# nihaomiao/WACV23_TSNet

Measured on AMD Instinct MI355X. Metric: retargeted frames/sec at bs=4, 256x256, n_source=3; max-abs delta vs ref, higher is better.
Workload: dtype f32 (convolutions: fp16 x 2 split of the scaled fp32 operands, 3 exact MFMA products, two-level fp32 accumulate; fp32-class accuracy); 1 GPU; TSNet(label_nc=2,n_blocks=0,n_downsampling=3,n_source=3) forward, fp32, B=4 per GPU, 256x256 (BASELINE.json configs[1]); global_batch=4, parallelism=replicas x1 (batch-sharded, weights broadcast once)

## Files before the change

include/tsnet_abi.h:

```cpp
#ifndef TSNET_ABI_H
#define TSNET_ABI_H

#include <stddef.h>
#include <stdint.h>

#ifdef __cplusplus
extern "C" {
#endif

#define TSNET_ABI_VERSION 5
#define TSNET_MAX_SOURCES 8

enum {
    TSNET_OK = 0,
    TSNET_ERR_ARG = -1,
    TSNET_ERR_WEIGHT = -2,
    TSNET_ERR_HIP = -3,
    TSNET_ERR_NOMEM = -4
};

typedef struct tsnet_engine* tsnet_handle;

typedef struct tsnet_cfg {
    int label_nc;
// ... 122 lines not shown
                       float* y, float* alpha, float* beta, void* stream);
int tsnet_op_finalize_stats(const double* part, int N, int S, int C, int HW, float* alpha, float* beta, void* stream);
int tsnet_op_fuse_tail(const float* src_fea, const float* tar_fea, const float* y2, const float* alpha, const float* beta,
                       int B, int K, int SB, int P, int C1, float* zbar, void* stream);
int tsnet_op_flow_k_slots(const float* tar_fea, const float* src_fea, const float* tar_bbox, const float* src_bbox,
                          int B, int K, int h, int w, int C, int H, int W, float* flow, int variant, int repeat, float* ms_out,
                          const int* slots, int n_src, void* stream);
int tsnet_op_warp_k_slots(const float* src_fea, const float* flow, int B, int K, int h, int w, int C, float* out,
                          const int* slots, int n_src, void* stream);
int tsnet_op_add_stats_slots(const float* x, const float* add, int add_nmod, int N, int HW, int C,
                             float* y, float* alpha, float* beta, const int* slots, int n_src, void* stream);
int tsnet_op_fuse_tail_slots(const float* src_fea, const float* tar_fea, const float* y2, const float* alpha, const float* beta,
                             int B, int K, int P, int C1, float* zbar, const int* slots, int n_src, void* stream);
int tsnet_op_pack_input(const float* const* img, const float* const* lbl, int S, int B, int H, int W, int L, int nimg, int Cp, int coords,
                        const float* img_div, float* out, unsigned int* amax, void* stream);
int tsnet_op_pack_input_u8(const uint8_t* const* img, const uint8_t* const* lbl, const uint8_t* const* bbox, int S, int B, int H, int W, int L,
                           int nimg, int Cp, int coords, const float* img_div, const float* mean_bgr, float* out, float* bbox_out,
                           unsigned int* amax, void* stream);
int tsnet_op_upsample2x_st(const float* x, const float* alpha, const float* beta, int relu,
                           int N, int H, int W, int C, int x_bf16, int y_bf16, float* y, void* stream);
int tsnet_op_patch_warp(const float* const* src_img, const float* div, const float* flow, int K, int B, int H, int W, int h, int w, float* out,
                        void* stream);
int tsnet_op_train_tail(float* x, const float* tar_img, const float* pg, const float* sg, int K, int B, int H, int W, int P, int C,
                        int fore_x0, int fore_x1, const float* bg, float* gen_mean, float* gen_std, float* ref_mean, float* ref_std,
                        float* losses, void* stream);
const char* tsnet_op_last_error(void);

int tsnet_frame_stats(const float* x, int B, int C, int HW, float div, float* mean, float* std_unbiased, void* stream);
int tsnet_demo_postprocess(const float* rec, int B, int H, int W, const float* gen_mean, const float* gen_std,
                           const float* ref_mean, const float* ref_std, const float* img_mean_over_255,
                           unsigned char* out_rgb, void* stream);

int tsnet_fit_face_curves(const double* keypoints, int F, double* curves);
int tsnet_raster_face(const double* keypoints, const double* curves, int F, int h, int w, int bw, unsigned char* edges, unsigned char* bbox, void* stream);
int tsnet_vl2ch(const float* labels, int B, int HW, int num_classes, float* out, void* stream);

int tsnet_face_adapt_stats(const double* kp, int F, double* stats);
int tsnet_face_adapt_apply(const double* stats, double* kp, int F);
int tsnet_smooth_keypoints(const double* in, int F, int P, double* out);

int tsnet_resize_label(const unsigned char* in, int F, int h, int w, int OH, int OW, const double* wts_rows, int lw_rows,
                       const double* wts_cols, int lw_cols, float* out, void* stream);
int tsnet_fit_pose_curves(const double* pts, int F, int flags, double* curves);
int tsnet_raster_pose(const double* pts, const double* curves, int F, int h, int w, int win_x0, int win_y0, int win_x1, int win_y1, int flags,
                      unsigned char* labels, void* stream);
int tsnet_label_bbox(const unsigned char* labels, int F, int h, int w, unsigned char* bbox, void* stream);
int tsnet_resize_pad(const unsigned char* in, int F, int h, int w, const int* ytab, const int* xtab, int oh, int ow,
                     int pad_top, int pad_left, int OH, int OW, int binarise, float* out, void* stream);

int tsnet_bench_conv(int N, int H, int W, int Cin, int Cout, int ksize, int stride, int pad, int pad_mode, int norm,
                     int variant, int iters, float* ms_out, void* stream);

void tsnet_debug_counters(int64_t out[4], int reset);

void tsnet_linspace(int n, float* out);
void tsnet_coord_table(int H, int W, float* out);

int tsnet_bicubic_taps(int n_in, int n_out);
int tsnet_bicubic_table(int n_in, int n_out, int* first, int* count, int* coef);
int tsnet_prepare_frames(const unsigned char* frames, int F, int h, int w, int x0, int y0, int x1, int y1,
                         const int* xfirst, const int* xcount, const int* xcoef, int xtaps,
                         const int* yfirst, const int* ycount, const int* ycoef, int ytaps,
                         int oh, int ow, int pad_top, int pad_left, int OH, int OW, const float* mean_bgr, float* out, void* stream);
int tsnet_prepare_frames_u8(const unsigned char* frames, int F, int h, int w, int x0, int y0, int x1, int y1,
                            const int* xfirst, const int* xcount, const int* xcoef, int xtaps,
                            const int* yfirst, const int* ycount, const int* ycoef, int ytaps,
                            int oh, int ow, int pad_top, int pad_left, int OH, int OW, unsigned char* out, void* stream);

int tsnet_paste_frames(const unsigned char* gen, const unsigned char* mask, int F, int GH, int GW, int sx0, int sy0, int sx1, int sy1,
                       const int* xfirst, const int* xcount, const int* xcoef, int xtaps,
                       const int* yfirst, const int* ycount, const int* ycoef, int ytaps,
                       unsigned char* frames, int h, int w, int x0, int y0, int x1, int y1, void* stream);

int tsnet_prepare_frames_boxes(const unsigned char* frames, int F, int h, int w, const int* boxes_host, const int* boxes_dev,
                               const int* pool, int pool_len, int oh, int ow, int pad_top, int pad_left, int OH, int OW,
                               const float* mean_bgr, float* out, void* stream);
int tsnet_prepare_frames_boxes_u8(const unsigned char* frames, int F, int h, int w, const int* boxes_host, const int* boxes_dev,
                                  const int* pool, int pool_len, int oh, int ow, int pad_top, int pad_left, int OH, int OW,
                                  unsigned char* out, void* stream);
int tsnet_paste_frames_boxes(const unsigned char* gen, const unsigned char* mask, int F, int GH, int GW, int sx0, int sy0, int sx1, int sy1,
                             const int* boxes_host, const int* boxes_dev, const int* pool, int pool_len,
                             unsigned char* frames, int h, int w, void* stream);

int tsnet_face_labels_boxes(const double* keypoints, const double* curves, int F, const int* desc_host, const int* desc_dev,
                            const double* pool, int pool_len, int bw, void* workspace, long long workspace_len, int OH, int OW,
                            float* labels, float* masks, void* stream);
int tsnet_face_labels_boxes_u8(const double* keypoints, const double* curves, int F, const int* desc_host, const int* desc_dev,
                               const double* pool, int pool_len, int bw, void* workspace, long long workspace_len, int OH, int OW,
                               unsigned char* labels, unsigned char* masks, void* stream);

int tsnet_gaussian_box_params(float radius, int passes, int* box_radius, unsigned* ww, unsigned* fw);
int tsnet_blur_mask(const unsigned char* in, int F, int H, int W, const int* rect, float radius_x, float radius_y, int flags,
                    unsigned char* out, unsigned char* tmp, void* stream);

#ifdef __cplusplus
}
#endif
#endif
```

wacv23_tsnet_amd/_lib.py:

```python
from __future__ import annotations

import ctypes as C
import os

import torch

_HERE = os.path.dirname(os.path.abspath(__file__))
LIB_PATH = os.path.join(_HERE, "lib", "libtsnet_hip.so")
MAX_SOURCES = 8
TIMING_CLASSES = 9
TIMING_NAMES = ("conv", "stats", "elementwise", "flow", "warp", "pack", "upsample", "other", "conv_res")

ABI_SYMBOLS = (
    "tsnet_abi_version", "tsnet_create", "tsnet_load_weights", "tsnet_finalize", "tsnet_destroy",
    "tsnet_last_error", "tsnet_num_params", "tsnet_param_info", "tsnet_packed_weights",
    "tsnet_forward", "tsnet_set_source_divisors", "tsnet_set_sources", "tsnet_set_sources_shared", "tsnet_forward_target", "tsnet_train_extras", "tsnet_stage_ptr",
    "tsnet_forward_macs", "tsnet_timing_enable", "tsnet_timing_read",
    "tsnet_op_conv2d", "tsnet_op_conv2d_cat", "tsnet_op_head", "tsnet_op_instnorm_stats", "tsnet_op_norm_act", "tsnet_op_upsample2x",
    "tsnet_op_flow", "tsnet_op_flow_k", "tsnet_flow_plan", "tsnet_op_warp", "tsnet_op_warp_k", "tsnet_op_warp_k_shared", "tsnet_op_add_stats", "tsnet_op_finalize_stats", "tsnet_op_fuse_tail", "tsnet_op_pack_input", "tsnet_op_upsample2x_st", "tsnet_op_last_error", "tsnet_frame_stats", "tsnet_demo_postprocess", "tsnet_fit_face_curves", "tsnet_raster_face", "tsnet_vl2ch", "tsnet_fit_pose_curves", "tsnet_raster_pose", "tsnet_label_bbox", "tsnet_resize_pad", "tsnet_resize_label", "tsnet_bench_conv", "tsnet_debug_counters", "tsnet_linspace", "tsnet_coord_table",
    "tsnet_bicubic_taps", "tsnet_bicubic_table", "tsnet_prepare_frames",
    "tsnet_face_adapt_stats", "tsnet_face_adapt_apply", "tsnet_smooth_keypoints",
    "tsnet_bank_capacity", "tsnet_bank_put", "tsnet_forward_bank",
    "tsnet_op_flow_k_slots", "tsnet_op_warp_k_slots", "tsnet_op_add_stats_slots", "tsnet_op_fuse_tail_slots",
    "tsnet_forward_u8", "tsnet_set_sources_u8", "tsnet_forward_target_u8", "tsnet_bank_put_u8", "tsnet_forward_bank_u8",
    "tsnet_op_pack_input_u8", "tsnet_prepare_frames_u8",
    "tsnet_paste_frames",
    "tsnet_prepare_frames_boxes", "tsnet_prepare_frames_boxes_u8", "tsnet_paste_frames_boxes",
    "tsnet_face_labels_boxes", "tsnet_face_labels_boxes_u8",
    "tsnet_op_upconv2d", "tsnet_op_conv2d_epi",
    "tsnet_op_patch_warp", "tsnet_op_train_tail",
    "tsnet_gaussian_box_params", "tsnet_blur_mask",
)


class TsnetCfg(C.Structure):
    _fields_ = [
        ("label_nc", C.c_int), ("n_blocks", C.c_int), ("n_downsampling", C.c_int), ("n_source", C.c_int),
        ("ngf", C.c_int), ("enc_blocks", C.c_int), ("addcoords", C.c_int), ("pose_composite", C.c_int),
        ("pose_mean", C.c_float * 3), ("height", C.c_int), ("width", C.c_int), ("max_batch", C.c_int), ("operand_mode", C.c_int),
    ]


_fp = C.POINTER(C.c_float)
_vp = C.c_void_p
CONV_EPI_INFO = 8


class TsnetConvEpi(C.Structure):
    _fields_ = [
        ("stats", C.c_int), ("repeat", C.c_int), ("part", _vp), ("part_capacity", C.c_longlong), ("alpha", _vp), ("beta", _vp),
        ("counters", _vp), ("counters_nonzero_out", C.POINTER(C.c_int)), ("addend", _vp), ("add_nmod", C.c_int), ("amax_out", _vp),
        ("in_amax", _vp), ("bound_add", C.c_float), ("x_bf16", C.c_int), ("y_bf16", C.c_int), ("info_out", C.POINTER(C.c_int)),
    ]


def bind(lib: C.CDLL) -> C.CDLL:
    lib.tsnet_abi_version.restype = C.c_int
    lib.tsnet_create.argtypes = [C.POINTER(TsnetCfg), C.POINTER(_vp)]
    lib.tsnet_load_weights.argtypes = [_vp, C.c_char_p, _vp, C.POINTER(C.c_int64), C.c_int]
    lib.tsnet_finalize.argtypes = [_vp, _vp]
    lib.tsnet_destroy.argtypes = [_vp]
    lib.tsnet_destroy.restype = None
    lib.tsnet_last_error.argtypes = [_vp]
    lib.tsnet_last_error.restype = C.c_char_p
    lib.tsnet_num_params.argtypes = [_vp]
    lib.tsnet_param_info.argtypes = [_vp, C.c_int, C.POINTER(C.c_char_p), C.POINTER(C.c_int64), C.POINTER(C.c_int)]
    lib.tsnet_packed_weights.argtypes = [_vp, C.POINTER(_vp), C.POINTER(C.c_size_t)]
    pp = C.POINTER(_vp)
    lib.tsnet_forward.argtypes = [_vp, pp, pp, pp, _vp, _vp, _vp, _vp, C.c_int, _vp]
    lib.tsnet_set_source_divisors.argtypes = [_vp, _fp, C.c_int]
    lib.tsnet_set_sources.argtypes = [_vp, pp, pp, pp, C.c_int, _vp]
    if hasattr(lib, "tsnet_set_sources_shared"):
        lib.tsnet_set_sources_shared.argtypes = [_vp, pp, pp, pp, _vp]
    lib.tsnet_forward_target.argtypes = [_vp, _vp, _vp, _vp, _vp, C.c_int, _vp]
    lib.tsnet_train_extras.argtypes = [_vp, pp, _vp, C.c_int, _vp, _vp, _vp]
    lib.tsnet_stage_ptr.argtypes = [_vp, C.c_char_p, C.POINTER(_vp), C.POINTER(C.c_size_t)]
    lib.tsnet_forward_macs.argtypes = [_vp, C.c_int]
    lib.tsnet_forward_macs.restype = C.c_double
    lib.tsnet_timing_enable.argtypes = [_vp, C.c_int]
    lib.tsnet_timing_read.argtypes = [_vp, C.POINTER(C.c_double), C.POINTER(C.c_int64), C.c_int]
    lib.tsnet_op_conv2d.argtypes = [_vp, C.c_int, C.c_int, C.c_int, C.c_int, _vp, _vp, C.c_int, C.c_int, C.c_int,
                                    C.c_int, C.c_int, _vp, _vp, C.c_int, C.c_float, C.c_int, C.c_int, C.c_int, _vp, _vp]
    lib.tsnet_op_conv2d_cat.argtypes = [_vp, _vp] + [C.c_int] * 6 + [_vp, _vp] + [C.c_int] * 5 + [C.c_float, C.c_int, _vp, _vp]
    lib.tsnet_op_head.argtypes = [_vp, C.c_int, C.c_int, C.c_int, C.c_int, _vp, _vp, _vp, _vp, C.c_int, _fp, _vp, _vp]
    lib.tsnet_op_instnorm_stats.argtypes = [_vp, C.c_int, C.c_int, C.c_int, _vp, _vp, _vp]
    lib.tsnet_op_norm_act.argtypes = [_vp, _vp, _vp, C.c_int, _vp, C.c_int, C.c_int, C.c_int, _vp, _vp]
    lib.tsnet_op_upsample2x.argtypes = [_vp, _vp, _vp, C.c_int, C.c_int, C.c_int, C.c_int, C.c_int, _vp, _vp]
    lib.tsnet_resize_label.argtypes = [_vp, C.c_int, C.c_int, C.c_int, C.c_int, C.c_int, _vp, C.c_int, _vp, C.c_int, _vp, _vp]
    lib.tsnet_op_flow.argtypes = [_vp, _vp, _vp, _vp, C.c_int, C.c_int, C.c_int, C.c_int, C.c_int, C.c_int, _vp, _vp]
    lib.tsnet_op_flow_k.argtypes = [_vp, _vp, _vp, _vp] + [C.c_int] * 7 + [_vp, C.c_int, C.c_int, _fp, _vp]
    lib.tsnet_flow_plan.argtypes = [C.c_int] * 4
    lib.tsnet_op_warp.argtypes = [_vp, _vp, C.c_int, C.c_int, C.c_int, C.c_int, _vp, _vp]
    if hasattr(lib, "tsnet_op_warp_k"):
        lib.tsnet_op_warp_k.argtypes = [_vp, _vp] + [C.c_int] * 5 + [_vp, C.c_int, _fp, _vp]
    if hasattr(lib, "tsnet_op_fuse_tail"):
        lib.tsnet_op_warp_k_shared.argtypes = [_vp, _vp] + [C.c_int] * 6 + [_vp, _vp]
        lib.tsnet_op_add_stats.argtypes = [_vp, _vp] + [C.c_int] * 5 + [_vp, _vp, _vp, _vp]
        lib.tsnet_op_finalize_stats.argtypes = [_vp] + [C.c_int] * 4 + [_vp, _vp, _vp]
        lib.tsnet_op_fuse_tail.argtypes = [_vp] * 5 + [C.c_int] * 5 + [_vp, _vp]
        lib.tsnet_op_pack_input.argtypes = [pp, pp] + [C.c_int] * 8 + [_fp, _vp, _vp, _vp]
        lib.tsnet_op_upsample2x_st.argtypes = [_vp, _vp, _vp] + [C.c_int] * 7 + [_vp, _vp]
    lib.tsnet_op_last_error.restype = C.c_char_p
    lib.tsnet_frame_stats.argtypes = [_vp, C.c_int, C.c_int, C.c_int, C.c_float, _vp, _vp, _vp]
    lib.tsnet_demo_postprocess.argtypes = [_vp, C.c_int, C.c_int, C.c_int, _vp, _vp, _vp, _vp, _fp, _vp, _vp]
    lib.tsnet_fit_face_curves.argtypes = [_vp, C.c_int, _vp]
    lib.tsnet_fit_pose_curves.argtypes = [_vp, C.c_int, C.c_int, _vp]
    lib.tsnet_raster_face.argtypes = [_vp, _vp, C.c_int, C.c_int, C.c_int, C.c_int, _vp, _vp, _vp]
    lib.tsnet_vl2ch.argtypes = [_vp, C.c_int, C.c_int, C.c_int, _vp, _vp]
    lib.tsnet_raster_pose.argtypes = [_vp, _vp] + [C.c_int] * 8 + [_vp, _vp]
    lib.tsnet_label_bbox.argtypes = [_vp, C.c_int, C.c_int, C.c_int, _vp, _vp]
    lib.tsnet_resize_pad.argtypes = [_vp, C.c_int, C.c_int, C.c_int, _vp, _vp] + [C.c_int] * 7 + [_vp, _vp]
    lib.tsnet_bench_conv.argtypes = [C.c_int] * 12 + [_fp, _vp]
    lib.tsnet_debug_counters.argtypes = [C.POINTER(C.c_int64), C.c_int]
    lib.tsnet_debug_counters.restype = None
    lib.tsnet_linspace.argtypes = [C.c_int, _fp]
    lib.tsnet_linspace.restype = None
    lib.tsnet_coord_table.argtypes = [C.c_int, C.c_int, _fp]
    lib.tsnet_coord_table.restype = None
    if hasattr(lib, "tsnet_prepare_frames"):
        lib.tsnet_bicubic_taps.argtypes = [C.c_int, C.c_int]
        lib.tsnet_bicubic_table.argtypes = [C.c_int, C.c_int, _vp, _vp, _vp]
        lib.tsnet_prepare_frames.argtypes = [_vp] + [C.c_int] * 7 + [_vp, _vp, _vp, C.c_int, _vp, _vp, _vp, C.c_int] + [C.c_int] * 6 + [_fp, _vp, _vp]
    if hasattr(lib, "tsnet_face_adapt_stats"):
        lib.tsnet_face_adapt_stats.argtypes = [_vp, C.c_int, _vp]
        lib.tsnet_face_adapt_apply.argtypes = [_vp, _vp, C.c_int]
        lib.tsnet_smooth_keypoints.argtypes = [_vp, C.c_int, C.c_int, _vp]
    if hasattr(lib, "tsnet_forward_bank"):
        _ip = C.POINTER(C.c_int)
        lib.tsnet_bank_capacity.argtypes = [_vp]
        lib.tsnet_bank_put.argtypes = [_vp, C.c_int, C.c_int, pp, pp, pp, _fp, _vp]
        lib.tsnet_forward_bank.argtypes = [_vp, _ip, C.c_int, _vp, _vp, _vp, _vp, C.c_int, _vp]
        lib.tsnet_op_flow_k_slots.argtypes = [_vp, _vp, _vp, _vp] + [C.c_int] * 7 + [_vp, C.c_int, C.c_int, _fp, _ip, C.c_int, _vp]
        lib.tsnet_op_warp_k_slots.argtypes = [_vp, _vp] + [C.c_int] * 5 + [_vp, _ip, C.c_int, _vp]
        lib.tsnet_op_add_stats_slots.argtypes = [_vp, _vp] + [C.c_int] * 4 + [_vp, _vp, _vp, _ip, C.c_int, _vp]
        lib.tsnet_op_fuse_tail_slots.argtypes = [_vp] * 5 + [C.c_int] * 4 + [_vp, _ip, C.c_int, _vp]
    if hasattr(lib, "tsnet_forward_u8"):
        _ip = C.POINTER(C.c_int)
        lib.tsnet_forward_u8.argtypes = [_vp, pp, pp, pp, _vp, _vp, _fp, _vp, _vp, C.c_int, _vp]
        lib.tsnet_set_sources_u8.argtypes = [_vp, pp, pp, pp, _fp, C.c_int, C.c_int, _vp]
        lib.tsnet_forward_target_u8.argtypes = [_vp, _vp, _vp, _vp, _vp, C.c_int, _vp]
        lib.tsnet_bank_put_u8.argtypes = [_vp, C.c_int, C.c_int, pp, pp, pp, _fp, _fp, _vp]
        lib.tsnet_forward_bank_u8.argtypes = [_vp, _ip, C.c_int, _vp, _vp, _vp, _vp, C.c_int, _vp]
        lib.tsnet_op_pack_input_u8.argtypes = [pp, pp, pp] + [C.c_int] * 8 + [_fp, _fp, _vp, _vp, _vp, _vp]
        lib.tsnet_prepare_frames_u8.argtypes = [_vp] + [C.c_int] * 7 + [_vp, _vp, _vp, C.c_int, _vp, _vp, _vp, C.c_int] + [C.c_int] * 6 + [_vp, _vp]
    if hasattr(lib, "tsnet_paste_frames"):
        lib.tsnet_paste_frames.argtypes = [_vp, _vp] + [C.c_int] * 7 + [_vp, _vp, _vp, C.c_int, _vp, _vp, _vp, C.c_int] + [_vp] + [C.c_int] * 6 + [_vp]
    if hasattr(lib, "tsnet_paste_frames_boxes"):
        lib.tsnet_prepare_frames_boxes.argtypes = [_vp] + [C.c_int] * 3 + [_vp, _vp, _vp, C.c_int] + [C.c_int] * 6 + [_fp, _vp, _vp]
        lib.tsnet_prepare_frames_boxes_u8.argtypes = [_vp] + [C.c_int] * 3 + [_vp, _vp, _vp, C.c_int] + [C.c_int] * 6 + [_vp, _vp]
        lib.tsnet_paste_frames_boxes.argtypes = [_vp, _vp] + [C.c_int] * 7 + [_vp, _vp, _vp, C.c_int] + [_vp, C.c_int, C.c_int, _vp]
    if hasattr(lib, "tsnet_face_labels_boxes"):
        for fn in (lib.tsnet_face_labels_boxes, lib.tsnet_face_labels_boxes_u8):
            fn.argtypes = [_vp, _vp, C.c_int, _vp, _vp, _vp, C.c_int, C.c_int, _vp, C.c_longlong, C.c_int, C.c_int, _vp, _vp, _vp]
    if hasattr(lib, "tsnet_op_upconv2d"):
        lib.tsnet_op_upconv2d.argtypes = lib.tsnet_op_conv2d.argtypes
    if hasattr(lib, "tsnet_op_conv2d_epi"):
        lib.tsnet_op_conv2d_epi.argtypes = lib.tsnet_op_conv2d.argtypes[:-1] + [C.POINTER(TsnetConvEpi), _vp]
    if hasattr(lib, "tsnet_op_train_tail"):
        lib.tsnet_op_patch_warp.argtypes = [pp, _fp, _vp] + [C.c_int] * 6 + [_vp, _vp]
        lib.tsnet_op_train_tail.argtypes = [_vp] * 4 + [C.c_int] * 8 + [_fp] + [_vp] * 6
    if hasattr(lib, "tsnet_blur_mask"):
        lib.tsnet_gaussian_box_params.argtypes = [C.c_float, C.c_int, C.POINTER(C.c_int), C.POINTER(C.c_uint), C.POINTER(C.c_uint)]
        lib.tsnet_blur_mask.argtypes = [_vp, C.c_int, C.c_int, C.c_int, _vp, C.c_float, C.c_float, C.c_int, _vp, _vp, _vp]
    return lib


_cached = None
# ... 26 lines not shown
```

wacv23_tsnet_amd/csrc/conv_g64.hpp:

```cpp
#pragma once
#include "conv_common.hpp"

namespace tsnet {

constexpr int g64_group_pitch(int BM) { return BM * 32 + 64; }
constexpr int g64_plane_bytes(int BM) { return 4 * g64_group_pitch(BM); }
constexpr int g64_lds_bytes(int BM, int NPL, int Cin) { return 2 * NPL * g64_plane_bytes(BM) + 64 + 2 * Cin * 4; }

template <int KS, int BM, int NPROD, bool AFFINE>
__global__ __launch_bounds__(BM * 4, 1)
void conv_g64_kernel(ConvArgs a) {
    constexpr int BN = 128, WARPS_N = 4, WARPS_M = BM / 64, NT = BM * 4;
    constexpr int MT = 2, NTL = 1;
    constexpr int RS = 2;
    static_assert(BM == 64 || BM == 128, "64 or 128 rows");
    constexpr bool ONEP = one_product(NPROD), F16P = NPROD == kNprodF16;
    static_assert(ONEP || NPROD == 3, "one (a bf16 or an fp16 plane) or three products");
    constexpr int NPL = ONEP ? 1 : 2;
    constexpr int GP = g64_group_pitch(BM), PLANE = g64_plane_bytes(BM), STAGE = NPL * PLANE;
    constexpr int OFF_TAB = 2 * STAGE + 64;

    HIP_DYNAMIC_SHARED(__attribute__((aligned(16))) unsigned char, smem_raw)
    const int tid = threadIdx.x;
    const int lane = tid & 63;
    const int wave = TSNET_UNIFORM(tid >> 6);
    const int wm0 = (wave / WARPS_N) * 64, wn0 = (wave % WARPS_N) * 32;
    const int li = lane & 31, lh = lane >> 5;

    const int bid = xcd_item(blockIdx.x, a.tiles_m * a.tiles_n);
    const int tile_m = bid / a.tiles_n, tile_n = bid - tile_m * a.tiles_n;
    const int n0 = tile_n * BN;
    const int hw = a.Ho * a.Wo;
    const int img = tile_m / a.tpi;
    const int r0 = (tile_m - img * a.tpi) * BM;
    float in_scale = a.in_scale, in_unscale = a.in_unscale;
    if (NPROD != 1 && a.in_amax) h2_device_scale(a.in_amax + img, a.in_bound_add, in_scale, in_unscale);

    const int C2 = a.Cin - a.Csplit;
    const size_t planew = (size_t)((a.nchunks + 1) / 2 * 2) * a.Npad * 16;
    const bool xb16 = NPROD == 1 && a.x_bf16 && !a.x2;
    const tsnet_brsrc_t rsx = tsnet_make_brsrc(a.x, (unsigned)((size_t)a.N * a.H * a.W * a.Csplit * (xb16 ? 2 : 4)));
    const tsnet_brsrc_t rsx2 = tsnet_make_brsrc(a.x2 ? a.x2 : a.x, a.x2 ? (unsigned)((size_t)a.x2_nmod * a.H * a.W * C2 * 4) : 0u);
    tsnet_brsrc_t rsw[NPL];
#pragma unroll
    for (int p = 0; p < NPL; ++p) rsw[p] = tsnet_make_brsrc(a.w + p * planew, (unsigned)(planew * 2));

    float* tab = reinterpret_cast<float*>(smem_raw + OFF_TAB);
    if (AFFINE) {
        for (int c = tid; c < a.Cin; c += NT) {
            tab[c] = a.in_alpha[(size_t)img * a.Cin + c] * in_scale;
            tab[a.Cin + c] = a.in_beta[(size_t)img * a.Cin + c] * in_scale;
        }
    }

    const int q8 = tid & 7;
    const int srow0 = tid >> 3;
    bool s_valid[RS];
    int s_oy[RS], s_ox[RS];
    unsigned lds_w[RS];
#pragma unroll
    for (int s = 0; s < RS; ++s) {
        const int row = srow0 + s * (BM / 2);
        s_valid[s] = r0 + row < hw;
        const int rem = s_valid[s] ? r0 + row : 0;
// ... 31 lines not shown
            if (second) {
                const unsigned v = ok ? (unsigned)(((pix2 + iy * a.W + ix) * C2 + (cb - a.Csplit) + q8 * 4) * 4) : kOOB;
                ar[s][0] = TSNET_BUF_LOAD16(rsx2, v, 0u); ar[s][1] = TSNET_BUF_LOAD16(rsx2, v, 128u);
            } else if (xb16) {
                const unsigned v = ok ? (unsigned)(((pix0 + iy * a.W + ix) * a.Csplit + cb + q8 * 4) * 2) : kOOB;
#pragma unroll
                for (int h = 0; h < 2; ++h) {
                    const F2 p = TSNET_BUF_LOAD8(rsx, v, (unsigned)(h * 64));
                    const unsigned w0 = __builtin_bit_cast(unsigned, p.v[0]), w1 = __builtin_bit_cast(unsigned, p.v[1]);
                    ar[s][h].v[0] = __builtin_bit_cast(float, w0 << 16); ar[s][h].v[1] = __builtin_bit_cast(float, w0 & 0xFFFF0000u);
                    ar[s][h].v[2] = __builtin_bit_cast(float, w1 << 16); ar[s][h].v[3] = __builtin_bit_cast(float, w1 & 0xFFFF0000u);
                }
            } else {
                const unsigned v = ok ? (unsigned)(((pix0 + iy * a.W + ix) * a.Csplit + cb + q8 * 4) * 4) : kOOB;
                ar[s][0] = TSNET_BUF_LOAD16(rsx, v, 0u); ar[s][1] = TSNET_BUF_LOAD16(rsx, v, 128u);
            }
        }
    };
    auto store_a = [&](int stage, int cb) __attribute__((always_inline)) {
        unsigned char* base = smem_raw + stage * STAGE;
#pragma unroll
        for (int s = 0; s < RS; ++s) {
#pragma unroll
            for (int h = 0; h < 2; ++h) {
                float t[4];
                if (AFFINE) {
                    const F4 al = *reinterpret_cast<const F4*>(tab + cb + h * 32 + q8 * 4), be = *reinterpret_cast<const F4*>(tab + a.Cin + cb + h * 32 + q8 * 4);
#pragma unroll
                    for (int e = 0; e < 4; ++e) t[e] = __builtin_fmaxf(__builtin_fmaf(ar[s][h].v[e], al.v[e], be.v[e]), relu_floor) * am[s];
                } else {
#pragma unroll
                    for (int e = 0; e < 4; ++e) t[e] = __builtin_fmaxf(ar[s][h].v[e] * in_scale, relu_floor);
                }
                unsigned char* dst = base + lds_w[s] + h * 2 * GP;
                if (ONEP) {
                    uint2 w;
                    w.x = cvt_pk_one<F16P>(t[0], t[1]); w.y = cvt_pk_one<F16P>(t[2], t[3]);
                    *reinterpret_cast<uint2*>(dst) = w;
                } else {
                    unsigned h0, l0, h1, l1;
                    TSNET_SPLIT_2PAIRS(t[0], t[1], t[2], t[3], h0, l0, h1, l1);
                    uint2 hw2, lw2;
                    hw2.x = h0; hw2.y = h1; lw2.x = l0; lw2.y = l1;
                    *reinterpret_cast<uint2*>(dst) = hw2;
                    *reinterpret_cast<uint2*>(dst + PLANE) = lw2;
                }
            }
        }
    };

    const int a_off = (wm0 + li) * 32 + (lh ^ ((li >> 3) & 1)) * 16;
    const unsigned vB = (unsigned)((wn0 + li) * 32 + (lh ^ ((li >> 3) & 1)) * 16);
    F4 af[NPL][MT], bf[4][NPL];
    auto frag_a = [&](int stage, int g) __attribute__((always_inline)) {
#pragma unroll
        for (int p = 0; p < NPL; ++p)
#pragma unroll
            for (int i = 0; i < MT; ++i) af[p][i] = *reinterpret_cast<const F4*>(smem_raw + stage * STAGE + p * PLANE + g * GP + i * 1024 + a_off);
    };
    auto load_b = [&](int g, int kc) __attribute__((always_inline)) {
#pragma unroll
        for (int p = 0; p < NPL; ++p) bf[g][p] = TSNET_BUF_LOAD16(rsw[p], vB, (unsigned)((kc * a.Npad + n0) * 32));
    };

    f32x16 acc[MT], tot[MT];
#pragma unroll
    for (int i = 0; i < MT; ++i)
#pragma unroll
        for (int r = 0; r < 16; ++r) { acc[i][r] = 0.f; tot[i][r] = 0.f; }
    auto product = [&](int g, int pa, int pb, bool fresh) __attribute__((always_inline)) {
#pragma unroll
        for (int i = 0; i < MT; ++i) {
            f32x16 c = acc[i];
            if (fresh) {
#pragma unroll
                for (int r = 0; r < 16; ++r) c[r] = 0.f;
            }
            if (NPROD == 1) acc[i] = TSNET_MFMA_BF16(af[pa][i], bf[g][pb], c);
            else acc[i] = TSNET_MFMA_F16(af[pa][i], bf[g][pb], c);
        }
    };

    load_a();
    int cb_held = cur_c;
    if (AFFINE) __syncthreads();
    store_a(0, cb_held);
    load_a();
    cb_held = cur_c;
#pragma unroll
    for (int g = 0; g < 4; ++g) load_b(g, g);

    for (int st = 0; st < nsteps; ++st) {
        __syncthreads();
        const int stage = st & 1;
        store_a(stage ^ 1, cb_held);
        load_a();
        cb_held = cur_c;
#pragma unroll
        for (int g = 0; g < 4; ++g) {
            frag_a(stage, g);
            if (ONEP) {
                product(g, 0, 0, g == 0);
            } else {
                product(g, 1, 0, g == 0);
                product(g, 0, 1, false);
                product(g, 0, 0, false);
            }
            load_b(g, (st + 1) * 4 + g);
        }
#pragma unroll
        for (int i = 0; i < MT; ++i) tot[i] += acc[i];
    }

    const float unscale = a.w_unscale ? in_unscale * a.w_unscale[0] : in_unscale;
    f32x16 out[MT][NTL];
#pragma unroll
    for (int i = 0; i < MT; ++i)
#pragma unroll
        for (int r = 0; r < 16; ++r) out[i][0][r] = tot[i][r] * unscale;
    const int m_img = img * hw;
    __syncthreads();
    conv_epilogue<BN, WARPS_M, WARPS_N, MT, NTL>(a, out, smem_raw, tid, wave, n0, (size_t)tile_m,
                                                 [&](int l) { return r0 + l < hw ? m_img + r0 + l : -1; });
}

}
```

wacv23_tsnet_amd/csrc/conv_g64_launch.cpp:

```cpp
#include <stdexcept>

#include "conv_g64.hpp"
#include "conv_h2s32.hpp"
#include "head_mfma.hpp"
#include "kernels.hpp"

namespace tsnet {
namespace {

template <int KS, int BM, int NPROD>
void go(const ConvArgs& a, hipStream_t s) {
    launch_tiles(a.in_alpha ? conv_g64_kernel<KS, BM, NPROD, true> : conv_g64_kernel<KS, BM, NPROD, false>, BM * 4, (size_t)g64_lds_bytes(BM, one_product(NPROD) ? 1 : 2, a.Cin), a, s);
}

template <int NPROD>
void go_np(const ConvArgs& a, const ConvPlan& p, hipStream_t s) {
    if (a.taps == 1 && p.rows == 64) return go<1, 64, NPROD>(a, s);
    if (a.taps == 1 && p.rows == 128) return go<1, 128, NPROD>(a, s);
    if (a.taps == 9 && p.rows == 64) return go<3, 64, NPROD>(a, s);
    if (a.taps == 9 && p.rows == 128) return go<3, 128, NPROD>(a, s);
    plan_not_built(p, NPROD);
}

}

void launch_conv_g64(const ConvArgs& a, const ConvPlan& p, int nprod, hipStream_t s) {
    nprod == 3 ? go_np<3>(a, p, s) : (nprod == kNprodF16 ? go_np<kNprodF16>(a, p, s) : go_np<1>(a, p, s));
}

void launch_conv_h2s32(const ConvArgs& a, int nprod, hipStream_t s) {
    if (nprod == 3) launch_tiles(conv_h2s32_kernel<3>, 256, (size_t)h2s32_lds_bytes(2), a, s);
    else if (nprod == kNprodF16) launch_tiles(conv_h2s32_kernel<kNprodF16>, 256, (size_t)h2s32_lds_bytes(1), a, s);
    else launch_tiles(conv_h2s32_kernel<1>, 256, (size_t)h2s32_lds_bytes(1), a, s);
}

template <int TR>
static void go_head(const HeadMfmaArgs& a, hipStream_t s) {
    const size_t lds = head_mfma_lds_bytes(TR, a.C);
    ensure_dynamic_lds(reinterpret_cast<const void*>(head_mfma_kernel<TR>), lds);
    hipLaunchKernelGGL(head_mfma_kernel<TR>, dim3(((a.W + 31) / 32) * ((a.H + TR - 1) / TR), a.N), dim3(hm_threads(TR)), lds, s, a);
}

void launch_head_mfma(const HeadMfmaArgs& a, int rows, hipStream_t s) {
    if (rows == 32) go_head<32>(a, s);
    else if (rows == 16) go_head<16>(a, s);
    else if (rows == 8) go_head<8>(a, s);
    else throw std::logic_error("head_mfma: tile rows must be 8, 16 or 32");
}

void pack_head_mfma(const float* w_oihw_dev, int C, float scale, unsigned short* planes, hipStream_t s) {
    hipLaunchKernelGGL(pack_head_mfma_kernel, dim3(64), dim3(256), 0, s, w_oihw_dev, planes, C, scale);
}

}
```

wacv23_tsnet_amd/csrc/engine.cpp:

```cpp
#include <hip/hip_runtime.h>

#include <algorithm>
#include <cmath>
#include <cstdio>
#include <cstdlib>
#include <cstring>
#include <map>
#include <memory>
#include <stdexcept>
#include <string>
#include <vector>

#include "../../include/tsnet_abi.h"
#include "entry_common.hpp"
#include "conv_plan.hpp"
#include "kernels.hpp"
#include "flow_warp.hpp"
#include "head_conv.hpp"
#include "norm_elementwise.hpp"
#include "pack_weights.hpp"
#include "postproc.hpp"
#include "train_extras.hpp"

using namespace tsnet;
// ... 119 lines not shown

inline int conv_kpad(int ks, int cin_pad) { return round_up(ks * ks * cin_pad, KPAD_ALIGN); }
inline int conv_kpad_w1(int cin_pad) { return round_up(12 * cin_pad, KPAD_ALIGN); }
inline int conv_npad(int cout) { return cout >= 128 ? round_up(cout, 128) : round_up(cout, 64); }
inline int conv_cin_pad(int cin) { return cin <= 8 ? 8 : round_up(cin, 16); }

struct ConvCall {
    const float* x = nullptr; const float* x2 = nullptr;
    int csplit = 0, x2_nmod = 1;
    const float* alpha = nullptr; const float* beta = nullptr; int relu = 0;
    float bound = 0.f;
    const unsigned* in_amax = nullptr; float bound_add = 0.f;
    int N = 0, H = 0, W = 0;
    float* y = nullptr;
    const float* addend = nullptr; int add_nmod = 1;
    double* stat_part = nullptr; mutable int stat_S = 0;
    float* fin_alpha = nullptr; float* fin_beta = nullptr; int* fin_counter = nullptr;
    unsigned* amax_out = nullptr;
    int x_bf16 = 0, y_bf16 = 0;
    int nprod = 3;
    int tclass = TSNET_T_CONV;
    bool up2 = false;
};

inline int h2_scale_log2(float bound, int lim = 24) {
    if (!(bound > 0.f) || !std::isfinite(bound)) throw ArgError("conv: the operand bound must be positive and finite");
    int e = 0;
    (void)std::frexp(bound, &e);
    int sa = 15 - e;
    if (sa > lim) sa = lim;
    if (sa < -lim) sa = -lim;
    return sa;
}

ConvShape conv_shape(const ConvLayer& L, const ConvCall& c) {
    const bool f16 = c.nprod == TSNET_NPROD_F16;
    ConvShape sh;
    sh.ks = L.ks; sh.stride = L.stride; sh.pad = L.pad; sh.reflect = L.reflect; sh.cin = L.cin_pad; sh.cout = L.cout; sh.npad = L.npad; sh.kpad = L.kpad;
    sh.form = L.form; sh.N = c.N; sh.H = c.H; sh.W = c.W; sh.csplit = c.x2 ? c.csplit : 0; sh.x2_nmod = c.x2_nmod > 0 ? c.x2_nmod : 1;
    sh.transform = c.alpha != nullptr; sh.nprod = f16 ? 1 : c.nprod; sh.f16 = f16; sh.fin_counter = c.stat_part && c.fin_counter;
    sh.up2 = c.up2; sh.x_bf16 = c.x_bf16 != 0;
    return sh;
}

void run_conv(Ctx& ctx, const ConvLayer& L, const ConvCall& c, ConvRequest req = {}) {
    const bool bf16 = c.nprod == 1, f16 = c.nprod == TSNET_NPROD_F16;
    if (!L.wq) throw ArgError("conv: layer has no packed weights");
    if (c.alpha && !c.beta) throw ArgError("conv: alpha without beta");
    if ((c.x_bf16 || c.y_bf16) && !bf16) throw ArgError("conv: bf16 storage goes with bf16 operands");
    if (c.x_bf16 && c.x2) throw ArgError("conv: bf16 storage of a concatenated input is not built");
    if (c.x2 && c.csplit == 0) throw ArgError("conv: a second tensor needs a channel split");
#ifdef TSNET_TOOLS
    req.chunk_cap = g_tools_knob[0];
#endif
    if (c.up2 && (c.x_bf16 || c.y_bf16 || c.in_amax)) throw ArgError("conv: the fused x2 upsample takes fp32 tensors and an a-priori operand bound");
    const ConvShape sh = conv_shape(L, c);
    ConvPlan p;
    try { p = plan_conv(sh, req, ctx.cus); } catch (const std::invalid_argument& e) { throw ArgError(e.what()); }
    ConvArgs g{};
    g.x = c.x; g.x2 = c.x2; g.in_alpha = c.alpha; g.in_beta = c.alpha ? c.beta : nullptr; g.in_relu = c.relu;
    const int sa = (bf16 || c.in_amax) ? 0 : h2_scale_log2(L.form == 1 ? 2.f * c.bound : c.bound, f16 ? 64 : 24);
    g.in_scale = std::ldexp(1.0f, sa); g.in_unscale = std::ldexp(1.0f, -sa);
    g.in_amax = bf16 ? nullptr : c.in_amax; g.in_bound_add = c.bound_add; g.amax_out = c.amax_out;
    g.w = L.wq; g.w_unscale = bf16 ? nullptr : L.w_unscale; g.bias = L.bias; g.y = c.y;
    g.stat_part = c.stat_part; g.addend = c.addend; g.add_nmod = c.add_nmod > 0 ? c.add_nmod : 1;
    g.x_bf16 = c.x_bf16; g.y_bf16 = c.y_bf16;
    g.N = c.N; g.H = c.H; g.W = c.W; g.Cin = L.cin_pad; g.cin_log2 = ilog2(L.cin_pad);
    g.Csplit = c.x2 ? c.csplit : L.cin_pad; g.x2_nmod = sh.x2_nmod;
    g.Ho = sh.ho(); g.Wo = sh.wo();
    g.Cout = L.cout; g.Npad = L.npad; g.stride = L.stride; g.pad = L.pad; g.reflect = L.reflect;
    g.taps = L.form == 1 ? 12 : L.ks * L.ks; g.nchunks = (g.taps * g.Cin + 15) / 16; g.M = c.N * g.Ho * g.Wo;
    g.fin_alpha = c.fin_alpha; g.fin_beta = c.fin_beta; g.fin_eps = 1e-5f;
    g.tpi = p.tpi; g.tiles_m = p.tiles_m; g.tiles_n = p.tiles_n; g.fin_S = p.tpi; g.xcd_gn = p.xcd_gn;
    g.w1_chunk = p.w1_chunk; g.w1_tab2 = p.w1_tab2; g.fin_counter = p.fin ? c.fin_counter : nullptr;
    TimeScope ts(ctx, c.tclass);
    try {
        switch (p.family) {
        case ConvFamily::W1: launch_conv_w1(g, c.nprod, req.abl, ctx.stream); break;
        case ConvFamily::H2: launch_conv_h2(g, p, c.nprod, req.abl, req.opt, ctx.stream); break;
        case ConvFamily::H2S: launch_conv_h2s(g, c.nprod, ctx.stream); break;
        case ConvFamily::H2S32: launch_conv_h2s32(g, c.nprod, ctx.stream); break;
        case ConvFamily::H2D: launch_conv_h2d(g, p, c.nprod, ctx.stream); break;
        case ConvFamily::G64: launch_conv_g64(g, p, c.nprod, ctx.stream); break;
        case ConvFamily::H2R: launch_conv_h2r(g, p, c.nprod, ctx.stream); break;
        }
    } catch (const std::invalid_argument& e) { throw ArgError(e.what()); }
    ++g_launch_counters[p.family == ConvFamily::G64 || p.family == ConvFamily::H2R ? 1 : 0];
    if (c.tclass == TSNET_T_CONV_RES && plan_tile_code(p)) g_launch_counters[3] = plan_tile_code(p);
    check_launch("conv");
    c.stat_S = !c.stat_part ? 0 : (g.fin_counter ? -1 : g.tpi);
}

void run_stats(Ctx& ctx, const float* x, int N, int HW, int C, double* part, float* alpha, float* beta) {
    if (C & 3) throw ArgError("instnorm: C must be a multiple of 4");
    TimeScope ts(ctx, TSNET_T_STATS);
    const int cq = C / 4, cols = cq < 256 ? cq : 256, R = 256 / cols;
    int S = (HW + R * 8 - 1) / (R * 8);
    if (S > 64) S = 64;
    if (S < 1) S = 1;
    const int rps = (HW + S - 1) / S;
    S = (HW + rps - 1) / rps;
    StatsArgs sa{x, part, HW, C, S, rps};
    hipLaunchKernelGGL(in_stats_partial_kernel, dim3(S, N, (cq + 255) / 256), dim3(256), 0, ctx.stream, sa);
    check_launch("in_stats_partial");
    launch_finalize(part, alpha, beta, N, C, S, HW, ctx.stream);
}

void launch_finalize_impl(const double* part, float* alpha, float* beta, int N, int C, int S, int HW, hipStream_t s) {
    if (S > 8) {
        hipLaunchKernelGGL(in_finalize2_kernel, dim3((C + kFin2Ch - 1) / kFin2Ch, N), dim3(256), 0, s, part, alpha, beta, C, S, HW, 1e-5f);
    } else {
        const int NC = N * C;
        hipLaunchKernelGGL(in_finalize_kernel, dim3((NC + 255) / 256), dim3(256), 0, s, part, alpha, beta, NC, C, S, HW, 1e-5f);
    }
    check_launch("in_finalize");
}

void run_add_stats(Ctx& ctx, const float* x, const int* slot, const float* add, int add_nmod, float* y, int N, int HW, int C, double* part, float* alpha, float* beta) {
    if (C & 3) throw ArgError("add_stats: C must be a multiple of 4");
    TimeScope ts(ctx, TSNET_T_STATS);
    const int cq = C / 4, cols = cq < 256 ? cq : 256, R = 256 / cols;
    int S = (HW + R * 8 - 1) / (R * 8);
    if (S > 64) S = 64;
    if (S < 1) S = 1;
    const int rps = (HW + S - 1) / S;
    S = (HW + rps - 1) / rps;
    const int nmod = add_nmod > 0 ? add_nmod : 1;
    AddStatsArgs sa{x, slot, add, y, part, HW, C, S, rps, nmod};
    hipLaunchKernelGGL(add_stats_partial_kernel, dim3(S, N, (cq + 255) / 256), dim3(256), 0, ctx.stream, sa);
    check_launch("add_stats_partial");
    launch_finalize(part, alpha, beta, N, C, S, HW, ctx.stream);
}

void run_norm_act(Ctx& ctx, const float* x, const float* alpha, const float* beta, int relu, const float* resid,
                  int N, int HW, int C, float* y) {
    if (C & 3) throw ArgError("norm_act: C must be a multiple of 4");
// ... 1703 lines not shown

int tsnet_bench_conv(int N, int H, int W, int Cin, int Cout, int ksize, int stride, int pad, int pad_mode, int norm,
                     int variant, int iters, float* ms_out, void* stream) {
    OP_BEGIN
    if (iters < 1 || !ms_out) throw ArgError("bench_conv: bad argument");
    hipStream_t s = (hipStream_t)stream;
    Ctx ctx(s, current_device_cus());
    BenchVariant bv;
    try { bv = decode_bench_variant(variant); } catch (const std::invalid_argument& e) { throw ArgError(e.what()); }
    const int nprod = bv.nprod;
    const int Ho = (H + 2 * pad - ksize) / stride + 1, Wo = (W + 2 * pad - ksize) / stride + 1;
    const size_t xn = (size_t)N * H * W * Cin, yn = (size_t)N * Ho * Wo * Cout, wn = (size_t)Cout * Cin * ksize * ksize;
    DevBufs mem;
    float* x = mem.alloc<float>(xn * 4); float* y = mem.alloc<float>(yn * 4);
    float* al = mem.alloc<float>((size_t)N * Cin * 4); float* be = mem.alloc<float>((size_t)N * Cin * 4);
    std::vector<float> hbuf(std::max(std::max(xn, wn), (size_t)N * Cin));
    unsigned st = 12345u;
    auto fill = [&](float* d, size_t n, float scale, float off) {
        for (size_t i = 0; i < n; ++i) { st = st * 1664525u + 1013904223u; hbuf[i] = off + scale * ((float)(st >> 8) / 16777216.0f - 0.5f); }
        if (d) HIP_TRY(hipMemcpy(d, hbuf.data(), n * 4, hipMemcpyHostToDevice));
    };
    fill(x, xn, 2.f, 0.f); fill(al, (size_t)N * Cin, 1.f, 1.f); fill(be, (size_t)N * Cin, 0.5f, 0.f);
    fill(nullptr, wn, 0.1f, 0.f);
    {
        const int form = bv.form;
        OpLayer op(hbuf.data(), nullptr, Cin, Cout, ksize, stride, pad, pad_mode, nprod, s, form);
        std::vector<std::unique_ptr<OpLayer>> cold;
        if (bv.cold) for (int i = 0; i < 24; ++i) cold.emplace_back(new OpLayer(hbuf.data(), nullptr, Cin, Cout, ksize, stride, pad, pad_mode, nprod, s, form));
        ConvCall c; c.x = x; c.N = N; c.H = H; c.W = W; c.y = y; c.bound = (norm & 1) ? 64.f : 1.f; c.nprod = nprod;
        if (norm & 1) { c.alpha = al; c.beta = be; c.relu = 1; }
        if (norm & 2) {
            const size_t tpi = ((size_t)Ho * Wo + 63) / 64;
            c.stat_part = mem.alloc<double>(stat_part_doubles(N, tpi, Cout) * sizeof(double));
            c.fin_alpha = mem.alloc<float>((size_t)N * Cout * 4); c.fin_beta = mem.alloc<float>((size_t)N * Cout * 4);
            c.fin_counter = mem.alloc<int>(kFinCounterInts * sizeof(int));
            HIP_TRY(hipMemset(c.fin_counter, 0, kFinCounterInts * sizeof(int)));
        }
        for (int i = 0; i < 2; ++i) run_conv(ctx, op.L, c, bv.req);
        EventPair ev;
        HIP_TRY(hipEventRecord(ev.a, s));
        for (int i = 0; i < iters; ++i) run_conv(ctx, cold.empty() ? op.L : cold[(size_t)i % cold.size()]->L, c, bv.req);
        HIP_TRY(hipEventRecord(ev.b, s));
        *ms_out = ev.ms() / iters;
    }
    OP_END
}

#ifdef TSNET_TOOLS
void tsnet_tools_set(int key, int value) { if (key >= 0 && key < 8) g_tools_knob[key] = value; }
#endif
void tsnet_debug_counters(int64_t out[4], int reset) {
    for (int i = 0; i < 4; ++i) { if (out) out[i] = g_launch_counters[i]; if (reset && i < 3) g_launch_counters[i] = 0; }
}

void tsnet_linspace(int n, float* out) { linspace_pm1(n, out); }
void tsnet_coord_table(int H, int W, float* out) { coord_table(H, W, out); }

}

#define TSNET_ENGINE_CPP
#include "clip_entries.hpp"
```

wacv23_tsnet_amd/csrc/kernels.hpp:

```cpp
#pragma once
#include <hip/hip_runtime.h>

#include "conv_common.hpp"
#include "conv_plan.hpp"
#include "flow_args.hpp"

namespace tsnet {

void launch_conv_h2(const ConvArgs& a, const ConvPlan& p, int nprod, int abl, int opt, hipStream_t s);
void launch_conv_h2s(const ConvArgs& a, int nprod, hipStream_t s);
void launch_conv_h2d(const ConvArgs& a, const ConvPlan& p, int nprod, hipStream_t s);
void launch_conv_w1(const ConvArgs& a, int nprod, int abl, hipStream_t s);
void launch_conv_h2r(const ConvArgs& a, const ConvPlan& p, int nprod, hipStream_t s);
void launch_conv_g64(const ConvArgs& a, const ConvPlan& p, int nprod, hipStream_t s);
void launch_conv_h2s32(const ConvArgs& a, int nprod, hipStream_t s);

struct HeadMfmaArgs {
    const float* x;
    const float* alpha;
    const float* beta;
    const unsigned short* wq;
    const float* w_unscale;
    const float* bias;
    float* y;
    int N, H, W, C;
    int composite, fore_x0, fore_x1;
    float bg[3];
    int x_bf16;
    float in_scale, in_unscale;
};

constexpr size_t head_mfma_table_halves(int C) { return (size_t)(C / 8) * 40 * 2 * 64 * 8; }
void launch_head_mfma(const HeadMfmaArgs& a, int rows, hipStream_t s);
void pack_head_mfma(const float* w_oihw_dev, int C, float scale, unsigned short* planes, hipStream_t s);

void launch_flow_p(const FlowArgs& a, int variant, hipStream_t s);
void launch_flow(const FlowArgs& a, int NT, size_t lds, unsigned grid, hipStream_t s);

void ensure_dynamic_lds(const void* kernel, size_t bytes);
template <class Kernel>
void launch_tiles(Kernel k, int threads, size_t lds, const ConvArgs& a, hipStream_t s) {
    ensure_dynamic_lds(reinterpret_cast<const void*>(k), lds);
    hipLaunchKernelGGL(k, dim3(a.tiles_m * a.tiles_n), dim3(threads), lds, s, a);
}

}
```

Measured before the change: 873.9 frames/s.

## Add row-aligned stride-2 3x3 G64 conv schedule reusing loaded input rows across taps

Adds a specialised G64 conv path for the 3x3 stride-2 pad-1 layer with 64 input channels, used when the 64-output-pixel tile lies within one output row. For each kernel row it loads the input row once and serves the three horizontal taps from LDS by shifting the fragment offset. This replaces a per-tap im2col gather, cutting global loads and address arithmetic. It adds a kernel instantiation, a tools knob that forces the general path, and a debug launch counter, with some risk in the padding and edge-lane handling.

After: 876.5 frames/s, median of 6. Within noise of the previous version (+0.3%).

```diff
diff --git a/include/tsnet_abi.h b/include/tsnet_abi.h
--- a/include/tsnet_abi.h
+++ b/include/tsnet_abi.h
@@ -198,6 +198,7 @@
                      int variant, int iters, float* ms_out, void* stream);
 
 void tsnet_debug_counters(int64_t out[4], int reset);
+long long tsnet_debug_g64_row_aligned(int reset);
 
 void tsnet_linspace(int n, float* out);
 void tsnet_coord_table(int H, int W, float* out);
diff --git a/wacv23_tsnet_amd/_lib.py b/wacv23_tsnet_amd/_lib.py
--- a/wacv23_tsnet_amd/_lib.py
+++ b/wacv23_tsnet_amd/_lib.py
@@ -30,6 +30,7 @@
     "tsnet_op_upconv2d", "tsnet_op_conv2d_epi",
     "tsnet_op_patch_warp", "tsnet_op_train_tail",
     "tsnet_gaussian_box_params", "tsnet_blur_mask",
+    "tsnet_debug_g64_row_aligned",
 )
 
 
@@ -113,6 +114,9 @@
     lib.tsnet_bench_conv.argtypes = [C.c_int] * 12 + [_fp, _vp]
     lib.tsnet_debug_counters.argtypes = [C.POINTER(C.c_int64), C.c_int]
     lib.tsnet_debug_counters.restype = None
+    if hasattr(lib, "tsnet_debug_g64_row_aligned"):
+        lib.tsnet_debug_g64_row_aligned.argtypes = [C.c_int]
+        lib.tsnet_debug_g64_row_aligned.restype = C.c_longlong
     lib.tsnet_linspace.argtypes = [C.c_int, _fp]
     lib.tsnet_linspace.restype = None
     lib.tsnet_coord_table.argtypes = [C.c_int, C.c_int, _fp]
diff --git a/wacv23_tsnet_amd/csrc/conv_g64.hpp b/wacv23_tsnet_amd/csrc/conv_g64.hpp
--- a/wacv23_tsnet_amd/csrc/conv_g64.hpp
+++ b/wacv23_tsnet_amd/csrc/conv_g64.hpp
@@ -7,9 +7,11 @@
 constexpr int g64_plane_bytes(int BM) { return 4 * g64_group_pitch(BM); }
 constexpr int g64_lds_bytes(int BM, int NPL, int Cin) { return 2 * NPL * g64_plane_bytes(BM) + 64 + 2 * Cin * 4; }
 
-template <int KS, int BM, int NPROD, bool AFFINE>
-__global__ __launch_bounds__(BM * 4, 1)
-void conv_g64_kernel(ConvArgs a) {
+template <bool V> struct g64_flag { static constexpr bool value = V; };
+
+template <int KS, int BM, int NPROD, bool AFFINE, bool RA>
+__device__ __forceinline__ void conv_g64_body(const ConvArgs& a) {
+    static_assert(!RA || (KS == 3 && BM == 64), "the row-aligned schedule is the 3 x 3 layer's 64-row tile");
     constexpr int BN = 128, WARPS_N = 4, WARPS_M = BM / 64, NT = BM * 4;
     constexpr int MT = 2, NTL = 1;
     constexpr int RS = 2;
@@ -147,11 +149,11 @@
     const int a_off = (wm0 + li) * 32 + (lh ^ ((li >> 3) & 1)) * 16;
     const unsigned vB = (unsigned)((wn0 + li) * 32 + (lh ^ ((li >> 3) & 1)) * 16);
     F4 af[NPL][MT], bf[4][NPL];
-    auto frag_a = [&](int stage, int g) __attribute__((always_inline)) {
+    auto frag_a = [&](int stage, int g, int off) __attribute__((always_inline)) {
 #pragma unroll
         for (int p = 0; p < NPL; ++p)
 #pragma unroll
-            for (int i = 0; i < MT; ++i) af[p][i] = *reinterpret_cast<const F4*>(smem_raw + stage * STAGE + p * PLANE + g * GP + i * 1024 + a_off);
+            for (int i = 0; i < MT; ++i) af[p][i] = *reinterpret_cast<const F4*>(smem_raw + stage * STAGE + p * PLANE + g * GP + i * 1024 + off);
     };
     auto load_b = [&](int g, int kc) __attribute__((always_inline)) {
 #pragma unroll
@@ -176,6 +178,132 @@
         }
     };
 
+    if constexpr (RA) {
+    const int oy = r0 / a.Wo, x0 = r0 - oy * a.Wo;
+    const int esz = xb16 ? 2 : 4;
+    unsigned voff[RS], lds_ra[RS];
+#pragma unroll
+    for (int s = 0; s < RS; ++s) {
+        const int row = srow0 + s * 32;
+        voff[s] = (unsigned)((row * 128 + q8 * 4) * esz);
+        lds_ra[s] = (unsigned)((q8 >> 2) * GP + row * 32 + ((((q8 >> 1) & 1) ^ ((row >> 3) & 1)) * 16) + (q8 & 1) * 8);
+    }
+    const bool first = x0 == 0 && srow0 == 0;
+    const bool xlane = tid >= NT - 64 && tid < NT - 48;
+    const int xh = (tid >> 3) & 1;
+    const unsigned xvoff = (unsigned)((64 * 128 + xh * 32 + q8 * 4) * esz);
+    const unsigned xlds = (unsigned)((xh * 2 + (q8 >> 2)) * GP + 64 * 32 + ((q8 >> 1) & 1) * 16 + (q8 & 1) * 8);
+    const int a_off1 = (li + 1) * 32 + (lh ^ (((li + 1) >> 3) & 1)) * 16;
+    F4 ax;
+    float amx = 0.f;
+    bool pad_nx = false;
+#pragma unroll
+    for (int e = 0; e < 4; ++e) ax.v[e] = 0.f;
+    auto load_quad = [&](unsigned v, int h) __attribute__((always_inline)) {
+        F4 o;
+        if (xb16) {
+            const F2 p = TSNET_BUF_LOAD8(rsx, v, (unsigned)(h * 64));
+            const unsigned w0 = __builtin_bit_cast(unsigned, p.v[0]), w1 = __builtin_bit_cast(unsigned, p.v[1]);
+            o.v[0] = __builtin_bit_cast(float, w0 << 16); o.v[1] = __builtin_bit_cast(float, w0 & 0xFFFF0000u);
+            o.v[2] = __builtin_bit_cast(float, w1 << 16); o.v[3] = __builtin_bit_cast(float, w1 & 0xFFFF0000u);
+        } else {
+            o = TSNET_BUF_LOAD16(rsx, v, (unsigned)(h * 128));
+        }
+        return o;
+    };
+    auto load_ra = [&](int ky, bool odd) __attribute__((always_inline)) {
+        const int iy = 2 * oy - 1 + ky;
+        const bool row_ok = iy >= 0 && iy < a.H;
+        const unsigned pb = (unsigned)(((pix0 + iy * a.W + 2 * x0 - (odd ? 1 : 0)) * 64) * esz);
+        pad_nx = !row_ok || (odd && x0 == 0);
+#pragma unroll
+        for (int s = 0; s < RS; ++s) {
+            const bool ok = row_ok && !(odd && s == 0 && first);
+            am[s] = ok ? 1.f : 0.f;
+            const unsigned v = ok ? pb + voff[s] : kOOB;
+            ar[s][0] = load_quad(v, 0); ar[s][1] = load_quad(v, 1);
+        }
+        if (odd) {
+            amx = row_ok ? 1.f : 0.f;
+            if (xlane) ax = load_quad(row_ok ? pb + xvoff : kOOB, 0);
+        }
+    };
+    auto put = [&](const F4& x, int c0, float amv, auto padc, unsigned char* dst) __attribute__((always_inline)) {
+        constexpr bool PAD = decltype(padc)::value;
+        float t[4];
+        if (AFFINE) {
+            const F4 al = *reinterpret_cast<const F4*>(tab + c0), be = *reinterpret_cast<const F4*>(tab + 64 + c0);
+#pragma unroll
+            for (int e = 0; e < 4; ++e) {
+                const float u = __builtin_fmaxf(__builtin_fmaf(x.v[e], al.v[e], be.v[e]), relu_floor);
+                t[e] = PAD ? u * amv : u;
+            }
+        } else {
+#pragma unroll
+            for (int e = 0; e < 4; ++e) t[e] = __builtin_fmaxf(x.v[e] * in_scale, relu_floor);
+        }
+        if (ONEP) {
+            uint2 w;
+            w.x = cvt_pk_one<F16P>(t[0], t[1]); w.y = cvt_pk_one<F16P>(t[2], t[3]);
+            *reinterpret_cast<uint2*>(dst) = w;
+        } else {
+            unsigned h0, l0, h1, l1;
+            TSNET_SPLIT_2PAIRS(t[0], t[1], t[2], t[3], h0, l0, h1, l1);
+            uint2 hw2, lw2;
+            hw2.x = h0; hw2.y = h1; lw2.x = l0; lw2.y = l1;
+            *reinterpret_cast<uint2*>(dst) = hw2;
+            *reinterpret_cast<uint2*>(dst + PLANE) = lw2;
+        }
+    };
+    auto store_ra = [&](int stage, bool odd, auto padc) __attribute__((always_inline)) {
+        unsigned char* base = smem_raw + stage * STAGE;
+#pragma unroll
+        for (int s = 0; s < RS; ++s)
+#pragma unroll
+            for (int h = 0; h < 2; ++h) put(ar[s][h], h * 32 + q8 * 4, am[s], padc, base + lds_ra[s] + h * 2 * GP);
+        if (odd && xlane) put(ax, xh * 32 + q8 * 4, amx, padc, base + xlds);
+    };
+    auto store_held = [&](int stage, bool odd, bool pad) __attribute__((always_inline)) {
+        if (pad) store_ra(stage, odd, g64_flag<true>{});
+        else store_ra(stage, odd, g64_flag<false>{});
+    };
+
+    load_ra(0, true);
+    bool pad_held = pad_nx;
+    if (AFFINE) __syncthreads();
+    store_held(0, true, pad_held);
+    load_ra(0, false);
+    pad_held = pad_nx;
+#pragma unroll
+    for (int g = 0; g < 4; ++g) load_b(g, g);
+
+    int ky = 0, kx = 0;
+#pragma unroll 1
+    for (int st = 0; st < 9; ++st) {
+        __syncthreads();
+        const int stage = st & 1;
+        if (kx == 0 || (kx == 2 && ky < 2)) {
+            store_held(stage ^ 1, kx == 2, pad_held);
+            if (ky < 2) { load_ra(ky + 1, kx == 0); pad_held = pad_nx; }
+        }
+        const int off = kx == 2 ? a_off1 : a_off;
+#pragma unroll
+        for (int g = 0; g < 4; ++g) {
+            frag_a(stage, g, off);
+            if (ONEP) {
+                product(g, 0, 0, g == 0);
+            } else {
+                product(g, 1, 0, g == 0);
+                product(g, 0, 1, false);
+                product(g, 0, 0, false);
+            }
+            load_b(g, (st + 1) * 4 + g);
+        }
+#pragma unroll
+        for (int i = 0; i < MT; ++i) tot[i] += acc[i];
+        if (++kx == 3) { kx = 0; ++ky; }
+    }
+    } else {
     load_a();
     int cb_held = cur_c;
     if (AFFINE) __syncthreads();
@@ -193,7 +321,7 @@
         cb_held = cur_c;
 #pragma unroll
         for (int g = 0; g < 4; ++g) {
-            frag_a(stage, g);
+            frag_a(stage, g, a_off);
             if (ONEP) {
                 product(g, 0, 0, g == 0);
             } else {
@@ -206,6 +334,7 @@
 #pragma unroll
         for (int i = 0; i < MT; ++i) tot[i] += acc[i];
     }
+    }
 
     const float unscale = a.w_unscale ? in_unscale * a.w_unscale[0] : in_unscale;
     f32x16 out[MT][NTL];
@@ -219,4 +348,17 @@
                                                  [&](int l) { return r0 + l < hw ? m_img + r0 + l : -1; });
 }
 
+template <int KS, int BM, int NPROD, bool AFFINE>
+__global__ __launch_bounds__(BM * 4, 1)
+void conv_g64_kernel(ConvArgs a) { conv_g64_body<KS, BM, NPROD, AFFINE, false>(a); }
+
+template <int NPROD, bool AFFINE>
+__global__ __launch_bounds__(256, 1)
+void conv_g64_s2_kernel(ConvArgs a) { conv_g64_body<3, 64, NPROD, AFFINE, true>(a); }
+
+inline bool g64_row_aligned(const ConvArgs& a, int rows) {
+    return a.taps == 9 && rows == 64 && a.stride == 2 && a.pad == 1 && !a.reflect && !a.x2 && a.Cin == 64 && a.Csplit == 64 && a.W == 2 * a.Wo &&
+           a.Wo % 64 == 0;
 }
+
+}
diff --git a/wacv23_tsnet_amd/csrc/conv_g64_launch.cpp b/wacv23_tsnet_amd/csrc/conv_g64_launch.cpp
--- a/wacv23_tsnet_amd/csrc/conv_g64_launch.cpp
+++ b/wacv23_tsnet_amd/csrc/conv_g64_launch.cpp
@@ -13,8 +13,14 @@
     launch_tiles(a.in_alpha ? conv_g64_kernel<KS, BM, NPROD, true> : conv_g64_kernel<KS, BM, NPROD, false>, BM * 4, (size_t)g64_lds_bytes(BM, one_product(NPROD) ? 1 : 2, a.Cin), a, s);
 }
 
+int64_t g_row_aligned_launches = 0;
+
 template <int NPROD>
-void go_np(const ConvArgs& a, const ConvPlan& p, hipStream_t s) {
+void go_np(const ConvArgs& a, const ConvPlan& p, bool general, hipStream_t s) {
+    if (!general && g64_row_aligned(a, p.rows)) {
+        ++g_row_aligned_launches;
+        return launch_tiles(a.in_alpha ? conv_g64_s2_kernel<NPROD, true> : conv_g64_s2_kernel<NPROD, false>, 256, (size_t)g64_lds_bytes(64, one_product(NPROD) ? 1 : 2, a.Cin), a, s);
+    }
     if (a.taps == 1 && p.rows == 64) return go<1, 64, NPROD>(a, s);
     if (a.taps == 1 && p.rows == 128) return go<1, 128, NPROD>(a, s);
     if (a.taps == 9 && p.rows == 64) return go<3, 64, NPROD>(a, s);
@@ -24,8 +30,14 @@
 
 }
 
-void launch_conv_g64(const ConvArgs& a, const ConvPlan& p, int nprod, hipStream_t s) {
-    nprod == 3 ? go_np<3>(a, p, s) : (nprod == kNprodF16 ? go_np<kNprodF16>(a, p, s) : go_np<1>(a, p, s));
+void launch_conv_g64(const ConvArgs& a, const ConvPlan& p, int nprod, bool general, hipStream_t s) {
+    nprod == 3 ? go_np<3>(a, p, general, s) : (nprod == kNprodF16 ? go_np<kNprodF16>(a, p, general, s) : go_np<1>(a, p, general, s));
+}
+
+int64_t conv_g64_row_aligned_launches(bool reset) {
+    const int64_t n = g_row_aligned_launches;
+    if (reset) g_row_aligned_launches = 0;
+    return n;
 }
 
 void launch_conv_h2s32(const ConvArgs& a, int nprod, hipStream_t s) {
diff --git a/wacv23_tsnet_amd/csrc/engine.cpp b/wacv23_tsnet_amd/csrc/engine.cpp
--- a/wacv23_tsnet_amd/csrc/engine.cpp
+++ b/wacv23_tsnet_amd/csrc/engine.cpp
@@ -195,6 +195,9 @@
     if (c.x2 && c.csplit == 0) throw ArgError("conv: a second tensor needs a channel split");
 #ifdef TSNET_TOOLS
     req.chunk_cap = g_tools_knob[0];
+    const bool g64_general = g_tools_knob[3] != 0;
+#else
+    const bool g64_general = false;
 #endif
     if (c.up2 && (c.x_bf16 || c.y_bf16 || c.in_amax)) throw ArgError("conv: the fused x2 upsample takes fp32 tensors and an a-priori operand bound");
     const ConvShape sh = conv_shape(L, c);
@@ -224,7 +227,7 @@
         case ConvFamily::H2S: launch_conv_h2s(g, c.nprod, ctx.stream); break;
         case ConvFamily::H2S32: launch_conv_h2s32(g, c.nprod, ctx.stream); break;
         case ConvFamily::H2D: launch_conv_h2d(g, p, c.nprod, ctx.stream); break;
-        case ConvFamily::G64: launch_conv_g64(g, p, c.nprod, ctx.stream); break;
+        case ConvFamily::G64: launch_conv_g64(g, p, c.nprod, g64_general, ctx.stream); break;
         case ConvFamily::H2R: launch_conv_h2r(g, p, c.nprod, ctx.stream); break;
         }
     } catch (const std::invalid_argument& e) { throw ArgError(e.what()); }
@@ -2034,6 +2037,7 @@
 void tsnet_debug_counters(int64_t out[4], int reset) {
     for (int i = 0; i < 4; ++i) { if (out) out[i] = g_launch_counters[i]; if (reset && i < 3) g_launch_counters[i] = 0; }
 }
+long long tsnet_debug_g64_row_aligned(int reset) { return conv_g64_row_aligned_launches(reset != 0); }
 
 void tsnet_linspace(int n, float* out) { linspace_pm1(n, out); }
 void tsnet_coord_table(int H, int W, float* out) { coord_table(H, W, out); }
diff --git a/wacv23_tsnet_amd/csrc/kernels.hpp b/wacv23_tsnet_amd/csrc/kernels.hpp
--- a/wacv23_tsnet_amd/csrc/kernels.hpp
+++ b/wacv23_tsnet_amd/csrc/kernels.hpp
@@ -12,7 +12,8 @@
 void launch_conv_h2d(const ConvArgs& a, const ConvPlan& p, int nprod, hipStream_t s);
 void launch_conv_w1(const ConvArgs& a, int nprod, int abl, hipStream_t s);
 void launch_conv_h2r(const ConvArgs& a, const ConvPlan& p, int nprod, hipStream_t s);
-void launch_conv_g64(const ConvArgs& a, const ConvPlan& p, int nprod, hipStream_t s);
+void launch_conv_g64(const ConvArgs& a, const ConvPlan& p, int nprod, bool general, hipStream_t s);
+int64_t conv_g64_row_aligned_launches(bool reset);
 void launch_conv_h2s32(const ConvArgs& a, int nprod, hipStream_t s);
 
 struct HeadMfmaArgs {
```
